# uzh-rpg/dagr

Measured on AMD Instinct MI355X. Metric: events_per_sec, higher is better.
Workload: dtype f32; 1 GPU; dagr-s + --use_image --img_net resnet50, 640x480 synthetic S-uniform, B=8 windows/step x 100000 events (50 ms each), r=7, K=16, events->graph->GNN(+image fusion)->decoded head outputs->confidence mask + NMS (device); image_branch=in-line, engines=3

## Files before the change

### dagr_amd/csrc/dense.hip

```cpp
#include "common.hpp"

namespace dagr {
namespace {

__global__ __launch_bounds__(kBlock) void k_dense_winner(const int32_t *__restrict__ n_ptr, int n_max,
                                                        const float *__restrict__ pos,
                                                        const int32_t *__restrict__ batch, float vx, float vy, int B,
                                                        int Hc, int Wc, int32_t *__restrict__ winner,
                                                        int32_t *__restrict__ status) {
    const int n_nodes = n_ptr ? min(*n_ptr, n_max) : n_max;
    const int n = blockIdx.x * kBlock + threadIdx.x;
    if (n >= n_nodes) return;
    const int cx = (int)(pos[3 * n] / vx), cy = (int)(pos[3 * n + 1] / vy), b = batch[n];
    if (cx < 0 || cx >= Wc || cy < 0 || cy >= Hc || b < 0 || b >= B) { atomicOr(status, 1); return; }
    atomicMax(&winner[(b * Hc + cy) * Wc + cx], n);
}

__global__ __launch_bounds__(kBlock) void k_dense_write(int B, int C, int Hc, int Wc,
                                                       const int32_t *__restrict__ winner,
                                                       const float *__restrict__ x, int ldx,
                                                       float *__restrict__ dense) {
    const int gid = blockIdx.x * kBlock + threadIdx.x;
    if (gid >= B * C * Hc * Wc) return;
    const int cx = gid % Wc, cy = (gid / Wc) % Hc, ch = (gid / (Wc * Hc)) % C, b = gid / (Wc * Hc * C);
// ... 69 lines not shown
namespace {
__global__ __launch_bounds__(kBlock) void k_bn_relu_maxpool(const float *__restrict__ x, int B, int H, int W, int C,
                                                           const float *__restrict__ scale,
                                                           const float *__restrict__ shift, float *__restrict__ y,
                                                           int OH, int OW) {
    const int C4 = C >> 2;
    const int64_t total = (int64_t)B * OH * OW * C4;
    const int64_t gid = (int64_t)blockIdx.x * kBlock + threadIdx.x;
    if (gid >= total) return;
    const int c4 = (int)(gid % C4);
    int64_t r = gid / C4;
    const int ow = (int)(r % OW); r /= OW;
    const int oh = (int)(r % OH);
    const int b = (int)(r / OH);
    const float4 sc = reinterpret_cast<const float4 *>(scale)[c4], sh = reinterpret_cast<const float4 *>(shift)[c4];
    float4 m = make_float4(0.f, 0.f, 0.f, 0.f);
#pragma unroll
    for (int dy = 0; dy < 3; dy++) {
        const int ih = 2 * oh - 1 + dy;
        if (ih < 0 || ih >= H) continue;
#pragma unroll
        for (int dx = 0; dx < 3; dx++) {
            const int iw = 2 * ow - 1 + dx;
            if (iw < 0 || iw >= W) continue;
            const float4 v = reinterpret_cast<const float4 *>(x + (((size_t)b * H + ih) * W + iw) * C)[c4];
            m.x = fmaxf(m.x, v.x * sc.x + sh.x);
            m.y = fmaxf(m.y, v.y * sc.y + sh.y);
            m.z = fmaxf(m.z, v.z * sc.z + sh.z);
            m.w = fmaxf(m.w, v.w * sc.w + sh.w);
        }
    }
    reinterpret_cast<float4 *>(y + (((size_t)b * OH + oh) * OW + ow) * C)[c4] = m;
}
}
}

extern "C" int dagr_bn_relu_maxpool(const float *x_nhwc, int32_t B, int32_t H, int32_t W, int32_t C, const float *scale,
                                    const float *shift, float *y_nhwc, void *stream) {
    using namespace dagr;
    DAGR_CHECK_ARG(B >= 1 && H >= 1 && W >= 1 && C >= 4 && C % 4 == 0, "bad sizes (C must be a multiple of 4)");
    DAGR_CHECK_ARG(x_nhwc && scale && shift && y_nhwc, "NULL pointer");
    DAGR_CHECK_ARG(((uintptr_t)x_nhwc % 16) == 0 && ((uintptr_t)y_nhwc % 16) == 0 && ((uintptr_t)scale % 16) == 0 &&
                       ((uintptr_t)shift % 16) == 0, "buffers must be 16-byte aligned");
    const int OH = (H - 1) / 2 + 1, OW = (W - 1) / 2 + 1;
    const int64_t total = (int64_t)B * OH * OW * (C / 4);
    k_bn_relu_maxpool<<<(unsigned)ceil_div(total, (int64_t)kBlock), kBlock, 0, (hipStream_t)stream>>>(
        x_nhwc, B, H, W, C, scale, shift, y_nhwc, OH, OW);
    DAGR_CHECK_LAUNCH();
    return DAGR_OK;
}

namespace dagr {
namespace {
__global__ __launch_bounds__(kBlock) void k_bias_relu(float *__restrict__ y, const float *__restrict__ bias, int64_t n4,
                                                     int C4) {
    const int64_t stride = (int64_t)gridDim.x * kBlock;
    for (int64_t i = (int64_t)blockIdx.x * kBlock + threadIdx.x; i < n4; i += stride) {
        float4 a = reinterpret_cast<float4 *>(y)[i];
        const float4 b = reinterpret_cast<const float4 *>(bias)[i % C4];
        a.x += b.x; a.y += b.y; a.z += b.z; a.w += b.w;
        a.x = a.x < 0.f ? 0.f : a.x;
        a.y = a.y < 0.f ? 0.f : a.y;
        a.z = a.z < 0.f ? 0.f : a.z;
        a.w = a.w < 0.f ? 0.f : a.w;
        reinterpret_cast<float4 *>(y)[i] = a;
    }
}
}
}

namespace dagr {
namespace {
__global__ __launch_bounds__(kBlock) void k_bias_silu(float *__restrict__ y, const float *__restrict__ bias, int64_t n4,
                                                     int C4) {
    const int64_t stride = (int64_t)gridDim.x * kBlock;
    for (int64_t i = (int64_t)blockIdx.x * kBlock + threadIdx.x; i < n4; i += stride) {
        float4 a = reinterpret_cast<float4 *>(y)[i];
        const float4 b = reinterpret_cast<const float4 *>(bias)[i % C4];
        a.x += b.x; a.y += b.y; a.z += b.z; a.w += b.w;
        a.x = a.x / (1.0f + expf(-a.x));
        a.y = a.y / (1.0f + expf(-a.y));
        a.z = a.z / (1.0f + expf(-a.z));
        a.w = a.w / (1.0f + expf(-a.w));
        reinterpret_cast<float4 *>(y)[i] = a;
    }
}
}
}

extern "C" int dagr_bias_silu(float *y_nhwc, const float *bias, int64_t n, int32_t C, void *stream) {
    using namespace dagr;
    DAGR_CHECK_ARG(n >= 0 && C >= 4 && C % 4 == 0 && n % C == 0, "bad sizes (C must be a multiple of 4 and divide n)");
    if (n == 0) return DAGR_OK;
    DAGR_CHECK_ARG(y_nhwc && bias, "NULL pointer");
    DAGR_CHECK_ARG(((uintptr_t)y_nhwc % 16) == 0 && ((uintptr_t)bias % 16) == 0, "buffers must be 16-byte aligned");
    const int64_t n4 = n >> 2;
    const int64_t blocks = ceil_div(n4, (int64_t)kBlock * 4);
    k_bias_silu<<<(unsigned)std::min<int64_t>(blocks, 256 * 16), kBlock, 0, (hipStream_t)stream>>>(y_nhwc, bias, n4, C / 4);
    DAGR_CHECK_LAUNCH();
    return DAGR_OK;
}

extern "C" int dagr_bias_relu(float *y_nhwc, const float *bias, int64_t n, int32_t C, void *stream) {
    using namespace dagr;
    DAGR_CHECK_ARG(n >= 0 && C >= 4 && C % 4 == 0 && n % C == 0, "bad sizes (C must be a multiple of 4 and divide n)");
    if (n == 0) return DAGR_OK;
// ... 9 lines not shown
```

### dagr_amd/csrc/gemm_lt.hip

```cpp
#include <hipblaslt/hipblaslt.h>

#include <map>
#include <tuple>

#include "common.hpp"

namespace dagr {
namespace {

struct LtPlan {
    hipblasLtMatmulDesc_t desc = nullptr;
    hipblasLtMatrixLayout_t a = nullptr, b = nullptr, c = nullptr, d = nullptr;
    hipblasLtMatmulAlgo_t algo;
    size_t workspace = 0;
};

hipblasLtHandle_t lt_handle() {
    static hipblasLtHandle_t h = [] {
        hipblasLtHandle_t hh = nullptr;
        if (hipblasLtCreate(&hh) != HIPBLAS_STATUS_SUCCESS) hh = nullptr;
        return hh;
    }();
    return h;
}

}
}

using namespace dagr;

extern "C" size_t dagr_gemm_epilogue_workspace_bytes(void) { return (size_t)64 << 20; }

extern "C" int dagr_gemm_epilogue(const float *A, int64_t M, int32_t K, int64_t lda, const float *Wt, int32_t N,
                                  const float *bias, const float *R, int64_t ldr, int32_t act, float *D, int64_t ldd,
                                  void *workspace, size_t workspace_bytes, void *stream) {
    DAGR_CHECK_ARG(M >= 0 && K >= 1 && N >= 1 && lda >= K && ldd >= N && (!R || ldr >= N) && (act == 0 || act == 1), "bad sizes");
    if (M == 0) return DAGR_OK;
    DAGR_CHECK_ARG(A && Wt && D, "NULL pointer");
    DAGR_CHECK_ARG((const float *)D != A, "D aliases A");
    DAGR_CHECK_ARG((const float *)D != R, "D aliases R");
    hipblasLtHandle_t h = lt_handle();
    if (!h) { set_error("dagr_gemm_epilogue: hipblasLtCreate failed"); return DAGR_ERR_HIP; }
    using Key = std::tuple<int64_t, int, int, int64_t, int64_t, int64_t, int, int, int>;
    static thread_local std::map<Key, LtPlan> plans;
    const Key key{M, K, N, lda, R ? ldr : -1, ldd, act, bias ? 1 : 0, R ? 1 : 0};
    auto it = plans.find(key);
    if (it == plans.end()) {
        LtPlan p;
#define LT_OK(expr)                                                                                        \
    do {                                                                                                   \
        if ((expr) != HIPBLAS_STATUS_SUCCESS) { set_error("dagr_gemm_epilogue: " #expr " failed"); return DAGR_ERR_HIP; } \
    } while (0)
        LT_OK(hipblasLtMatmulDescCreate(&p.desc, HIPBLAS_COMPUTE_32F, HIP_R_32F));
        const hipblasOperation_t op_n = HIPBLAS_OP_N;
        LT_OK(hipblasLtMatmulDescSetAttribute(p.desc, HIPBLASLT_MATMUL_DESC_TRANSA, &op_n, sizeof(op_n)));
        LT_OK(hipblasLtMatmulDescSetAttribute(p.desc, HIPBLASLT_MATMUL_DESC_TRANSB, &op_n, sizeof(op_n)));
        hipblasLtEpilogue_t epi = act ? (bias ? HIPBLASLT_EPILOGUE_RELU_BIAS : HIPBLASLT_EPILOGUE_RELU)
                                      : (bias ? HIPBLASLT_EPILOGUE_BIAS : HIPBLASLT_EPILOGUE_DEFAULT);
        LT_OK(hipblasLtMatmulDescSetAttribute(p.desc, HIPBLASLT_MATMUL_DESC_EPILOGUE, &epi, sizeof(epi)));
        if (bias) {
            const hipDataType bt = HIP_R_32F;
            LT_OK(hipblasLtMatmulDescSetAttribute(p.desc, HIPBLASLT_MATMUL_DESC_BIAS_DATA_TYPE, &bt, sizeof(bt)));
            LT_OK(hipblasLtMatmulDescSetAttribute(p.desc, HIPBLASLT_MATMUL_DESC_BIAS_POINTER, &bias, sizeof(bias)));
        }
        LT_OK(hipblasLtMatrixLayoutCreate(&p.a, HIP_R_32F, (uint64_t)N, (uint64_t)K, (int64_t)N));
        LT_OK(hipblasLtMatrixLayoutCreate(&p.b, HIP_R_32F, (uint64_t)K, (uint64_t)M, lda));
        LT_OK(hipblasLtMatrixLayoutCreate(&p.c, HIP_R_32F, (uint64_t)N, (uint64_t)M, R ? ldr : ldd));
        LT_OK(hipblasLtMatrixLayoutCreate(&p.d, HIP_R_32F, (uint64_t)N, (uint64_t)M, ldd));
        hipblasLtMatmulPreference_t pref = nullptr;
        LT_OK(hipblasLtMatmulPreferenceCreate(&pref));
        const uint64_t max_ws = workspace ? (uint64_t)workspace_bytes : 0;
        LT_OK(hipblasLtMatmulPreferenceSetAttribute(pref, HIPBLASLT_MATMUL_PREF_MAX_WORKSPACE_BYTES, &max_ws, sizeof(max_ws)));
        constexpr int kCand = 16;
        hipblasLtMatmulHeuristicResult_t res[kCand];
        int found = 0;
        const hipblasStatus_t st = hipblasLtMatmulAlgoGetHeuristic(h, p.desc, p.a, p.b, p.c, p.d, pref, kCand, res, &found);
        hipblasLtMatmulPreferenceDestroy(pref);
        if (st != HIPBLAS_STATUS_SUCCESS || found < 1) {
            set_error("dagr_gemm_epilogue: the library offers no kernel for this GEMM + epilogue");
            return DAGR_ERR_UNSUPPORTED;
        }
        int best = 0;
        hipStreamCaptureStatus cap = hipStreamCaptureStatusNone;
        (void)hipStreamIsCapturing((hipStream_t)stream, &cap);
        if (found > 1 && cap == hipStreamCaptureStatusNone) {
            hipEvent_t e0, e1;
            if (hipEventCreate(&e0) == hipSuccess && hipEventCreate(&e1) == hipSuccess) {
                const float alpha = 1.0f, beta = R ? 1.0f : 0.0f;
                float best_ms = 0.f;
                for (int c = 0; c < found; c++) {
                    if (res[c].workspaceSize > workspace_bytes) continue;
                    bool ok = true;
                    float ms = 0.f;
                    for (int rep = 0; rep < 3 && ok; rep++) {
                        if (rep == 1) (void)hipEventRecord(e0, (hipStream_t)stream);
                        ok = hipblasLtMatmul(h, p.desc, &alpha, Wt, p.a, A, p.b, &beta, R ? (const void *)R : (const void *)D,
                                             p.c, D, p.d, &res[c].algo, workspace, workspace_bytes,
                                             (hipStream_t)stream) == HIPBLAS_STATUS_SUCCESS;
                    }
                    (void)hipEventRecord(e1, (hipStream_t)stream);
                    if (hipEventSynchronize(e1) != hipSuccess || !ok) continue;
                    (void)hipEventElapsedTime(&ms, e0, e1);
                    if (best_ms == 0.f || ms < best_ms) { best_ms = ms; best = c; }
                }
                (void)hipEventDestroy(e0);
                (void)hipEventDestroy(e1);
            }
        }
        p.algo = res[best].algo;
        p.workspace = res[best].workspaceSize;
        it = plans.emplace(key, p).first;
#undef LT_OK
    }
    LtPlan &p = it->second;
    if (bias && hipblasLtMatmulDescSetAttribute(p.desc, HIPBLASLT_MATMUL_DESC_BIAS_POINTER, &bias, sizeof(bias)) !=
                    HIPBLAS_STATUS_SUCCESS) {
        set_error("dagr_gemm_epilogue: setting the bias pointer failed");
        return DAGR_ERR_HIP;
    }
    DAGR_CHECK_ARG(p.workspace <= workspace_bytes, "workspace too small for the selected kernel");
    const float alpha = 1.0f, beta = R ? 1.0f : 0.0f;
    const hipblasStatus_t st = hipblasLtMatmul(h, p.desc, &alpha, Wt, p.a, A, p.b, &beta, R ? (const void *)R : (const void *)D,
                                               p.c, D, p.d, &p.algo, workspace, workspace_bytes, (hipStream_t)stream);
    if (st != HIPBLAS_STATUS_SUCCESS) {
        set_error("dagr_gemm_epilogue: hipblasLtMatmul failed");
        return DAGR_ERR_HIP;
    }
    return DAGR_OK;
}
```

### dagr_amd/engine.py

```python
import contextlib
import ctypes
import gc
import types

import numpy as np
import torch

from . import _lib
from .graph.ev_graph import WindowGraphBuilder

FUSED_PASSES_MAX_NODES = 1600

L0_WIDTHS = (8, 16, 32)


def _l0_block(c):
    cm = max(b for b in (0,) + L0_WIDTHS if b <= c)
    return cm, c - cm


def _f32(v):
    return float(torch.as_tensor(v, dtype=torch.float32))


# ... 142 lines not shown


def _add_relu_(y, z):
    if y.is_cuda and y.dtype == torch.float32 and z.dtype == torch.float32 and y.shape == z.shape \
            and y.stride() == z.stride() and y.data_ptr() % 16 == 0 and z.data_ptr() % 16 == 0 \
            and (y.is_contiguous() or y.is_contiguous(memory_format=torch.channels_last)):
        _lib.check(_lib.lib().dagr_add_relu(_lib.ptr(y), _lib.ptr(z), y.numel(), _lib.cur_stream(y.device)), "add_relu")
        return y
    return torch.relu_(y.add_(z))


def _bias_relu_(y, bias):
    C = y.shape[1]
    if y.is_cuda and y.dtype == torch.float32 and C % 4 == 0 and y.is_contiguous(memory_format=torch.channels_last) \
            and y.data_ptr() % 16 == 0 and bias.data_ptr() % 16 == 0:
        _lib.check(_lib.lib().dagr_bias_relu(_lib.ptr(y), _lib.ptr(bias), y.numel(), C, _lib.cur_stream(y.device)),
                   "bias_relu")
        return y
    return torch.relu_(y.add_(bias.view(1, -1, 1, 1)))


def _baseconv_forward(m, x):
    y = m.conv(x)
    b = m._bias
    C = y.shape[1]
    if y.is_cuda and y.dtype == torch.float32 and C % 4 == 0 and y.is_contiguous(memory_format=torch.channels_last) \
            and y.data_ptr() % 16 == 0 and b.data_ptr() % 16 == 0:
        _lib.check(_lib.lib().dagr_bias_silu(_lib.ptr(y), _lib.ptr(b), y.numel(), C, _lib.cur_stream(y.device)),
                   "bias_silu")
        return y
    return torch.nn.functional.silu(y.add_(b.view(1, -1, 1, 1)), inplace=True)


def _conv_bias_relu(blk, name, x):
    conv = getattr(blk, name)
    b = getattr(blk, "_" + name + "_bias", None)
    out = conv(x)
    if b is not None:
        return _bias_relu_(out, b)
    if getattr(conv, "relu", False):
        return out
    return blk.relu(out)


def _bottleneck_forward(blk, x):
    identity = x if blk.downsample is None else blk.downsample(x)
    out = _conv_bias_relu(blk, "conv1", x)
    out = _conv_bias_relu(blk, "conv2", out)
    if isinstance(blk.conv3, _Conv1x1Gemm):
        return blk.conv3(out, residual=identity)
    return _add_relu_(blk.conv3(out), identity)


def _resnet_features_forward(net, x, emit=None):
    emit = emit or (lambda name, t: None)
    c1 = net.conv1(x)
    emit("conv1", c1)
    mp = net.maxpool
    ok = (c1.is_cuda and c1.dtype == torch.float32 and c1.is_contiguous(memory_format=torch.channels_last)
          and c1.shape[1] % 4 == 0 and mp.kernel_size == 3 and mp.stride == 2 and mp.padding == 1
          and mp.dilation == 1 and not mp.ceil_mode)
    if ok:
        B, C, H, W = c1.shape
        scale, shift = net._stem_affine
        y = torch.empty((B, C, (H - 1) // 2 + 1, (W - 1) // 2 + 1), dtype=c1.dtype, device=c1.device,
                        memory_format=torch.channels_last)
        _lib.check(_lib.lib().dagr_bn_relu_maxpool(_lib.ptr(c1), B, H, W, C, _lib.ptr(scale), _lib.ptr(shift), _lib.ptr(y),
                                                   _lib.cur_stream(c1.device)), "bn_relu_maxpool")
    else:
        y = net.maxpool(net.relu(net.bn1(c1)))
    l1 = net.layer1(y)
    emit("layer1", l1)
    l2 = net.layer2(l1)
    emit("layer2", l2)
    l3 = net.layer3(l2)
    emit("layer3", l3)
    l4 = net.layer4(l3)
    emit("layer4", l4)
    return dict(conv1=c1, layer1=l1, layer2=l2, layer3=l3, layer4=l4)


def _basicblock_forward(blk, x):
    identity = x if blk.downsample is None else blk.downsample(x)
    out = _conv_bias_relu(blk, "conv1", x)
    return _add_relu_(blk.conv2(out), identity)


class _Level:

    def __init__(self, T, cin, cout, device, cf_next=0):
        self.T = T
        self.e_cap = T * 64
        i32 = dict(dtype=torch.int32, device=device)
        f32 = dict(dtype=torch.float32, device=device)
        self.x = torch.zeros((T, (cin + 3) // 4 * 4), **f32)
        self.pos = torch.zeros((T, 3), **f32)
        self.batch = torch.zeros((T,), **i32)
        self.rowptr = torch.zeros((T + 2,), **i32)
        self.col = torch.zeros((self.e_cap,), **i32)
        self.code = torch.zeros((self.e_cap,), **i32)
        self.counts = torch.zeros((2,), **i32)
        self.cluster = torch.zeros((T,), **i32)
        self.h1 = torch.zeros((T, cout), **f32)
        self.hp = torch.zeros((T, cout + cf_next), **f32)
        self.cout = cout


class WindowEngine:
    def __init__(self, model, max_events=1 << 17, device="cuda"):
        self.model = model
        self.device = torch.device(device)
        args = model.args
        bb, head = model.backbone, model.head
        self.args = args
        self.B = int(args.batch_size)
        self.W, self.H = int(model.width), int(model.height)
        self.time_window = int(getattr(args, "time_window_us", 1000000))
        self.num_classes = bb.num_classes
        self.num_scales = int(args.num_scales)
        self.use_image = bool(args.use_image)
        self.no_events = bool(getattr(args, "no_events", False))
        self.feat_ch = list(bb.net.feature_channels) if self.use_image else [0] * 5
# ... 415 lines not shown

    def _fold_image_branch(self):
        import copy
        from torch.nn.utils.fusion import fuse_conv_bn_eval
        bb, head = self.model.backbone, self.model.head
        net = copy.deepcopy(bb.net).eval()
        cnn = copy.deepcopy(head.cnn_head).eval()

        def fold_block(blk):
            for ci, bi in (("conv1", "bn1"), ("conv2", "bn2"), ("conv3", "bn3")):
                if hasattr(blk, ci):
                    setattr(blk, ci, fuse_conv_bn_eval(getattr(blk, ci), getattr(blk, bi)))
                    setattr(blk, bi, torch.nn.Identity())
            if blk.downsample is not None:
                blk.downsample = torch.nn.Sequential(fuse_conv_bn_eval(blk.downsample[0], blk.downsample[1]))
        for name in ("layer1", "layer2", "layer3", "layer4"):
            for blk in getattr(net.module, name):
                fold_block(blk)
        for m in cnn.modules():
            if hasattr(m, "conv") and hasattr(m, "bn") and isinstance(m.bn, torch.nn.BatchNorm2d):
                m.conv = fuse_conv_bn_eval(m.conv, m.bn)
                m.bn = torch.nn.Identity()
                if isinstance(getattr(m, "act", None), torch.nn.SiLU) and m.conv.bias is not None:
                    m._bias = m.conv.bias.detach().clone().contiguous()
                    m.conv.bias = None
                    m.forward = types.MethodType(_baseconv_forward, m)
        net = net.to(memory_format=torch.channels_last)
        cnn = cnn.to(memory_format=torch.channels_last)
        for blkname in ("layer1", "layer2", "layer3", "layer4"):
            _gemmify_1x1(getattr(net.module, blkname))
            for blk in getattr(net.module, blkname):
                relu_convs = ("conv1", "conv2") if hasattr(blk, "conv3") else ("conv1",)
                for cname in relu_convs:
                    conv = getattr(blk, cname)
                    if isinstance(conv, _Conv1x1Gemm):
                        conv.relu = True
                    elif isinstance(conv, torch.nn.Conv2d) and conv.bias is not None:
                        setattr(blk, "_" + cname + "_bias", conv.bias.detach().clone().contiguous())
                        conv.bias = None
                blk.forward = types.MethodType(_bottleneck_forward if hasattr(blk, "conv3") else _basicblock_forward,
                                               blk)
        bn = net.module.bn1
        scale = (bn.weight.detach().float() / torch.sqrt(bn.running_var.detach().float() + bn.eps)).contiguous()
        shift = (bn.bias.detach().float() - bn.running_mean.detach().float() * scale).contiguous()
        net.module._stem_affine = (scale, shift)
        net.module.forward_features = types.MethodType(_resnet_features_forward, net.module)
        _gemmify_1x1(net.feature_dconv)
        _gemmify_1x1(net.output_dconv)
        self._net_f, self._cnn_f = net, cnn

    def _image_branch(self, image, on_feature=None):
        if self._net_f is None:
            self._fold_image_branch()
        bb, head = types.SimpleNamespace(net=self._net_f), types.SimpleNamespace(cnn_head=self._cnn_f)
        x = image.contiguous(memory_format=torch.channels_last)
        net = self._net_f
        if on_feature is not None:
            feats = [None] * len(net.feature_layers)

            def emit(name, t):
                if name in net.feature_layers:
                    j = net.feature_layers.index(name)
                    feats[j] = net.feature_dconv[j](t) if len(net.feature_dconv) > 0 else t
                    on_feature(j, feats[j])
            d = _resnet_features_forward(net.module, x, emit)
            outs = [d[l] for l in net.output_layers]
            if len(net.output_dconv) > 0:
                outs = [dconv(o) for o, dconv in zip(outs, net.output_dconv)]
        else:
            feats, outs = bb.net(x)
        outs = outs[-self.num_scales:]
        resized = [torch.nn.functional.interpolate(f, o) for f, o in zip(outs, self.out_sizes)]
        return feats, head.cnn_head(resized)

    def stage_image(self, image):
        self._keep = []
        self._img_feats, self._cnn_out = self._image_branch(image)

    def image_async(self, image, stream=None):
        cur = torch.cuda.current_stream(self.device)
        if stream is not None:
            self._img_stream = stream
        if self._img_stream is None:
            self._img_stream = torch.cuda.Stream(self.device)
        s = self._img_stream
        s.wait_stream(cur)
        with torch.cuda.stream(s):
            feats, cnn_out = self._image_branch(image)
            ev = torch.cuda.Event()
            ev.record(s)
        return feats, cnn_out, ev

    def _consume_image_handle(self, handle):
        feats, cnn_out, ev = handle
        cur = torch.cuda.current_stream(self.device)
        cur.wait_event(ev)
        for t in list(feats) + [o for v in cnn_out.values() for o in v]:
            t.record_stream(cur)
        self._keep = []
        self._img_feats, self._cnn_out = feats, cnn_out

    def stage_l0_input(self, feat):
        N = self._N
        x0 = self.x0buf[:N]
        g = self.graph
        if not self._inputs_gathered:
            f = feat.float().reshape(-1).contiguous()
            _lib.check(self.L.dagr_graph_gather_inputs(ctypes.byref(g.desc), _lib.ptr(g.workspace), _lib.ptr(self._pos),
                                                       _lib.ptr(f), N, _lib.ptr(self.pos_n), _lib.ptr(self.batch_n),
                                                       _lib.ptr(x0), self.x0_ld, self.x0_feat_col, self.x0_pos_col,
                                                       _lib.cur_stream(self.device)), "graph_gather_inputs")
        if self.use_image:
            self._sample(self._nptr(), N, self.pos_n, self.batch_n, 0, self._img_feats[0], x0, self.x0_img_col)
        self._x0 = x0

    def _conv_l0(self, pack, x, ldx, xskip, ldskip, out, ldo):
        L, P = self.L, _lib.ptr
        nbr_src, nbr_code, deg = self._nbr
        cin, cskip, w, s = pack
        d0 = self.dom[0]
        wx, tx, wy, ty = self.win0
        stream = _lib.cur_stream(self.device)
        if self.l0_tiles:
# ... 519 lines not shown
```

### include/dagr_hip.h

```cpp
#ifndef DAGR_HIP_H
#define DAGR_HIP_H

#include <stddef.h>
#include <stdint.h>

#ifdef __cplusplus
extern "C" {
#endif

typedef enum {
    DAGR_OK = 0,
    DAGR_ERR_INVALID_ARG = -1,
    DAGR_ERR_HIP = -2,
    DAGR_ERR_WORKSPACE = -3,
    DAGR_ERR_UNSUPPORTED = -4
} dagr_status;

const char *dagr_last_error(void);
int dagr_version(void);
int dagr_device_count(void);

int dagr_format_events(const int16_t *xy , const int32_t *t , const int8_t *p ,
                       int64_t N, int32_t width, int32_t height, int32_t time_window,
                       float *pos_out , float *feat_out , void *stream);
// ... 190 lines not shown
    const float *w2, *s2; float *hp0; int32_t ldhp0;
    const dagr_pool_desc *pdesc; void *pool_ws; const int32_t *xlo, *ylo;
    float *x_out; int32_t ldo; float *pos_out; int32_t *batch_out, *n_out, *rowptr_out, *col_out, *code_out, *e_out;
    int32_t e_cap;
} dagr_async_update_args;
int dagr_async_update(const dagr_async_update_args *args, void *stream);
int dagr_async_update_w(const dagr_async_update_args *args, int32_t cout0, void *stream);
int dagr_pool_l0_accumulate(const dagr_pool_desc *desc, void *pool_ws, const dagr_graph_desc *gdesc, void *graph_ws,
                            const int32_t *xlo, const int32_t *ylo, const float *x, int32_t ldx, const float *pos,
                            int64_t N, const int32_t *nbr_src, const int16_t *nbr_code, const int32_t *deg, void *stream);
int dagr_pool_l0_stream(const dagr_pool_desc *desc, void *pool_ws, int32_t rebuild, const dagr_graph_desc *gdesc,
                        void *graph_ws, const int32_t *xlo, const int32_t *ylo, const float *x, int32_t ldx, const float *pos,
                        const int32_t *batch_events, int64_t n_window, int64_t first_row, int64_t n_rows,
                        const int32_t *nbr_src, const int16_t *nbr_code, const int32_t *deg, float *x_out, int32_t ldo,
                        int32_t xoff, float *pos_out, int32_t *batch_out, int32_t *n_out, int32_t *rowptr_out,
                        int32_t *col_out, int32_t *code_out, int32_t *e_out, int32_t e_cap, void *stream);

int dagr_spline_conv_fused_pool(const int32_t *n_nodes_ptr, int32_t n_nodes_max, const int32_t *rowptr,
                                const int32_t *col, const int32_t *code, const float *x, int32_t ldx, int32_t cin,
                                const float *xskip, int32_t ldskip, int32_t cskip, int32_t rx, int32_t ry,
                                float den_x, float den_y, const float *Wq, const float *bias, float *C,
                                int32_t ldc, int32_t N, int32_t relu, const dagr_pool_desc *pdesc, void *pool_ws,
                                const float *pos, const int32_t *batch, int32_t *cluster_scratch, void *stream);
int dagr_pool_csr(const dagr_pool_desc *desc, void *pool_ws, const int32_t *n_ptr, int32_t n_max, const float *x,
                  int32_t ldx, const float *pos, const int32_t *batch, const int32_t *rowptr, const int32_t *col,
                  int32_t *cluster_scratch , float *x_out, int32_t ldo, int32_t xoff, float *pos_out,
                  int32_t *batch_out, int32_t *n_out, int32_t *rowptr_out, int32_t *col_out, int32_t *code_out,
                  int32_t *e_out, int32_t e_cap, void *stream);
int dagr_pool_recode(const int32_t *n_ptr, int32_t n_max, const int32_t *rowptr, const int32_t *col, const float *pos,
                     float two_max, float r00, float r02, float r11, float r12, int32_t rx, int32_t ry,
                     int32_t *code_out, int32_t e_cap, int32_t *status, void *stream);
int dagr_pool_status(const dagr_pool_desc *desc, void *pool_ws, int32_t *flags_host, void *stream);
const int32_t *dagr_pool_status_ptr(const dagr_pool_desc *desc, void *pool_ws);
int dagr_pool_counters(const dagr_pool_desc *desc, void *pool_ws, int32_t *out8_host, void *stream);

int dagr_to_dense(const int32_t *n_ptr, int32_t n_max, const float *x, int32_t ldx, int32_t channels,
                  const float *pos, const int32_t *batch, float vx, float vy, int32_t batch_size,
                  int32_t Hc, int32_t Wc, int32_t *winner_scratch, float *dense, int32_t *status, void *stream);

int dagr_pool_argmax(const int32_t *cluster, int32_t n, const float *x, int32_t ldx, int32_t channels,
                     const float *x_pooled, int32_t ldp, int32_t n_clusters, int32_t *arg, void *stream);
int dagr_pool_grad(const int32_t *cluster, int32_t n, int32_t channels, int32_t aggr, const int32_t *arg,
                   const int32_t *count, const float *grad_pooled, int32_t ldg, float *grad_x, int32_t ldgx,
                   void *stream);
int dagr_to_dense_grad(int32_t n, int32_t channels, const float *pos, const int32_t *batch, float vx, float vy,
                       int32_t batch_size, int32_t Hc, int32_t Wc, const float *grad_dense,
                       float *grad_x, int32_t ldgx, void *stream);

int dagr_add_relu(float *y, const float *z, int64_t n, void *stream);
int dagr_bias_relu(float *y_nhwc, const float *bias, int64_t n, int32_t C, void *stream);
int dagr_bias_silu(float *y_nhwc, const float *bias, int64_t n, int32_t C, void *stream);
int dagr_bn_relu_maxpool(const float *x_nhwc, int32_t B, int32_t H, int32_t W, int32_t C, const float *scale,
                         const float *shift, float *y_nhwc, void *stream);

int dagr_sample_features(const int32_t *n_ptr, int32_t n_max, const float *pos, const void *batch,
                         int32_t batch_is_int64, const float *feat_nhwc, int32_t B, int32_t h, int32_t w, int32_t C,
                         int32_t width, int32_t height, float *out, int32_t ldo, int32_t coff, void *stream);

int dagr_nms_batched(const float *boxes, const float *scores, const int32_t *cls, const uint8_t *valid,
                     int32_t B, int32_t A, float iou_threshold, float class_offset,
                     int32_t *order_out, int32_t *keep_out, int32_t *n_keep, void *stream);

typedef struct dagr_head_scale {
    const int32_t *n_ptr; int32_t n_max;
    const float *pred; int32_t ld;
    const float *pos; const int32_t *batch;
    float vx, vy, stride; int32_t Hc, Wc;
    const float *cnn[3]; int32_t cnn_stride[3][4];
    float *dense;
} dagr_head_scale;
int dagr_heads_finish(const dagr_head_scale *scale0, const dagr_head_scale *scale1, int32_t batch_size, int32_t channels,
                      float *out, int32_t *status, void *stream);
int dagr_heads_finish_detect(const dagr_head_scale *scale0, const dagr_head_scale *scale1, int32_t batch_size,
                             int32_t channels, float *out, int32_t *status, float conf_threshold, float iou_threshold,
                             float class_offset, float *det, int32_t *n_keep, void *stream);
int dagr_decode_heads(const float *dense0, int32_t H0, int32_t W0, float stride0, const float *dense1, int32_t H1,
                      int32_t W1, float stride1, int32_t B, int32_t channels, float *out, void *stream);

int dagr_postprocess(const float *pred, int32_t B, int32_t A, int32_t num_classes, float conf_threshold,
                     float iou_threshold, float class_offset, float *det, int32_t *n_keep, void *stream);

int dagr_masked_lin(const int64_t *indices, const float *x_in, float *x_out, const float *weight, const float *bias,
                    int32_t add, int64_t K, int32_t Cin, int32_t Cout, void *stream);
int dagr_masked_lin_no_bias(const int64_t *indices, const float *x_in, float *x_out, const float *weight, int32_t add,
                            int64_t K, int32_t Cin, int32_t Cout, void *stream);
int dagr_masked_isdiff(int64_t *indices, const float *x_old, const float *x_new, float atol, float rtol, int64_t K,
                       int32_t C, void *stream);
int dagr_masked_inplace_BN(const int64_t *indices, const float *x, float *x_out, const float *running_mean,
                           const float *running_var, const float *weight, const float *bias, float eps, int64_t K,
                           int32_t C, void *stream);

int dagr_downsample_events(const int32_t *order, const int32_t *run_cell, const int32_t *run_end, int32_t n_runs,
                           const int8_t *polarity, int32_t fx, int32_t fy, float *change_map, uint8_t *keep,
                           void *stream);

size_t dagr_gemm_epilogue_workspace_bytes(void);
int dagr_gemm_epilogue(const float *A, int64_t M, int32_t K, int64_t lda, const float *Wt, int32_t N, const float *bias,
                       const float *R, int64_t ldr, int32_t act, float *D, int64_t ldd, void *workspace,
                       size_t workspace_bytes, void *stream);

enum { DAGR_FLOPS_ZERO = 0, DAGR_FLOPS_CONV = 1, DAGR_FLOPS_LINEAR = 2, DAGR_FLOPS_POOL = 3, DAGR_FLOPS_CARTESIAN = 4 };
typedef struct dagr_flops_module {
    int32_t kind, level, cin, cout, root, bias;
} dagr_flops_module;
int dagr_async_flops(const int32_t *deg, int32_t n_events, const int32_t *counts1, const int32_t *counts2,
                     const int32_t *counts3, const int32_t *counts4, const dagr_flops_module *mods, int32_t n_mods,
                     int64_t *out, void *stream);

size_t dagr_viz_workspace_bytes(int32_t F, int32_t H, int32_t W);
int dagr_viz_render(const uint8_t *images, int32_t n_images, int32_t H, int32_t W, const int32_t *frame_image, int32_t F,
                    const int32_t *ev_x, const int32_t *ev_y, const int8_t *ev_p, const int32_t *ev_ptr, int32_t n_events,
                    const double *alpha, const int32_t *boxes, const int32_t *box_ptr, int32_t n_boxes, int32_t linewidth,
                    const uint8_t *colors, int32_t n_colors, uint8_t *out, int32_t *status, void *workspace,
                    size_t workspace_bytes, void *stream);

typedef struct dagr_aug_params {
    int32_t flip, crop_on;
    int32_t crop_lo[2], crop_hi[2];
    float zoom;
    int32_t move[2];
} dagr_aug_params;
size_t dagr_augment_workspace_bytes(int64_t N);
int dagr_augment_events(const dagr_aug_params *params, int32_t B, int32_t W, int32_t H, const void *pos, int32_t pos_width,
                        const void *t, int32_t t_width, const void *p, int32_t p_width, const int32_t *sample_ptr, int64_t N,
                        int16_t *out_pos, void *out_t, void *out_p, int64_t *out_batch, int32_t *out_ptr,
                        int32_t *status, void *workspace, size_t workspace_bytes, void *stream);
int dagr_augment_status(const int32_t *status, void *stream);
int dagr_augment_frames(const dagr_aug_params *params, int32_t B, int32_t C, int32_t H, int32_t W, int32_t elem_bytes,
                        int32_t reference_crop, const void *in, void *out, void *stream);
int dagr_augment_boxes(const dagr_aug_params *params, int32_t B, int32_t W, int32_t H, const float *boxes,
                       const int64_t *box_batch, int32_t M, int32_t ld, float *out, void *stream);

#define DAGR_COCO_MAX_GT 256
#define DAGR_COCO_MAX_DT 4096
#define DAGR_COCO_MAX_DETS 100
void dagr_coco_match_bounds(int32_t *max_gt, int32_t *max_dt, int32_t *max_dets);
int dagr_coco_match(const double *gt_xywh, const double *dt_xywh, const double *dt_score, const int64_t *jobs,
                    const double *area_rng, const double *iou_thrs, int32_t n_thr, int32_t max_dets, int64_t n_jobs,
                    int64_t n_gt, int64_t n_dt, int32_t max_gt_per_job, int32_t max_dt_per_job, int64_t n_out,
                    int64_t n_gign, int32_t *order, uint8_t *dtm, uint8_t *dt_ign, uint8_t *g_ign, int32_t *status,
                    void *stream);

#define DAGR_COCO_ACC_TILE 1024
#define DAGR_COCO_ACC_MAX_REC 128
int32_t dagr_coco_accumulate_tile(void);
size_t dagr_coco_accumulate_workspace_bytes(int32_t n_thr, int64_t n_cols);
int dagr_coco_accumulate(const uint8_t *dtm, const uint8_t *dt_ign, const int32_t *perm, const int64_t *group_ptr,
                         const int64_t *group_ngt, const double *rec_thrs, int32_t n_rec, double eps, int32_t n_thr,
                         int32_t n_groups, int64_t n_cols, void *workspace, size_t workspace_bytes, double *precision,
                         int32_t *status, void *stream);

int dagr_spiral_offsets(int32_t n, int32_t *dx_host, int32_t *dy_host);
// ... 6 lines not shown
```

Before: 147.5 million events/s.

## Fuse stem BN-ReLU-maxpool with conv1 projection and widen hipBLASLt algo search

New measurement: 148.4 million events/s, median of 6. About the same (+0.6%).

```diff
diff --git a/dagr_amd/csrc/dense.hip b/dagr_amd/csrc/dense.hip
--- a/dagr_amd/csrc/dense.hip
+++ b/dagr_amd/csrc/dense.hip
@@ -145,6 +145,169 @@
 
 namespace dagr {
 namespace {
+constexpr int kStemRows = 4, kStemCols = 32;
+constexpr int kStemLR = kStemRows + 1, kStemLC = kStemCols + 1;
+constexpr int kStemPix = kStemLR * kStemLC;
+constexpr int kStemMaxC = 64;
+constexpr int kStemLoads = (kStemPix * (kStemMaxC / 4) + kBlock - 1) / kBlock;
+
+template <int NT>
+__device__ __forceinline__ void stem_tile_compute(const float4 *l_x, const float4 *l_aff, int tile, int B, int H, int W,
+                                                  int C, float *__restrict__ y, int OH, int OW, const float *__restrict__ wd,
+                                                  const float *__restrict__ bd, int N, float *__restrict__ proj,
+                                                  int tiles_x, int tiles_y) {
+    const int C4 = C >> 2, ld4 = C4 + 1;
+    const int q_step = kBlock / C4, c_step = kBlock - q_step * C4;
+    const int q_first = (int)threadIdx.x / C4, c_first = (int)threadIdx.x - q_first * C4;
+    {
+        const int tx = tile % tiles_x, ty = (tile / tiles_x) % tiles_y, b = tile / (tiles_x * tiles_y);
+        const int r0 = ty * kStemRows - 1, c0 = tx * kStemCols - 1;
+
+        constexpr int kOwned = kStemRows * kStemCols;
+        for (int item = threadIdx.x; item < kOwned * (N / NT); item += kBlock) {
+            const int p = item & (kOwned - 1);
+            const int n0 = __builtin_amdgcn_readfirstlane(item / kOwned) * NT;
+            const int lr = 1 + p / kStemCols, lc = 1 + p % kStemCols;
+            const int ih = r0 + lr, iw = c0 + lc;
+            if (ih >= H || iw >= W) continue;
+            const float4 *src = l_x + (lr * kStemLC + lc) * ld4;
+            float acc[NT];
+#pragma unroll
+            for (int j = 0; j < NT; j++) acc[j] = 0.f;
+            for (int k4 = 0; k4 < C4; k4++) {
+                const float4 f = src[k4];
+                const float *w = wd + (size_t)(4 * k4) * N + n0;
+#pragma unroll
+                for (int j = 0; j < NT; j++) acc[j] = fmaf(f.x, w[j], acc[j]);
+#pragma unroll
+                for (int j = 0; j < NT; j++) acc[j] = fmaf(f.y, w[N + j], acc[j]);
+#pragma unroll
+                for (int j = 0; j < NT; j++) acc[j] = fmaf(f.z, w[2 * N + j], acc[j]);
+#pragma unroll
+                for (int j = 0; j < NT; j++) acc[j] = fmaf(f.w, w[3 * N + j], acc[j]);
+            }
+            float *out = proj + (((size_t)b * H + ih) * W + iw) * N + n0;
+#pragma unroll
+            for (int j = 0; j < NT; j += 4)
+                reinterpret_cast<float4 *>(out)[j >> 2] = make_float4(acc[j] + bd[n0 + j], acc[j + 1] + bd[n0 + j + 1],
+                                                                      acc[j + 2] + bd[n0 + j + 2], acc[j + 3] + bd[n0 + j + 3]);
+        }
+
+        constexpr int kPoolCols = kStemCols / 2, kPooled = (kStemRows / 2) * kPoolCols;
+        int q = q_first, c4 = c_first;
+        for (; q < kPooled; q += q_step) {
+            const int ohl = q / kPoolCols, owl = q % kPoolCols;
+            const int oh = ty * (kStemRows / 2) + ohl, ow = tx * kPoolCols + owl;
+            if (oh < OH && ow < OW) {
+                const float4 sc = l_aff[c4], sh = l_aff[C4 + c4];
+                float4 m = make_float4(0.f, 0.f, 0.f, 0.f);
+#pragma unroll
+                for (int dy = 0; dy < 3; dy++) {
+                    const int ih = 2 * oh - 1 + dy;
+#pragma unroll
+                    for (int dx = 0; dx < 3; dx++) {
+                        const int iw = 2 * ow - 1 + dx;
+                        const bool in = ih >= 0 && ih < H && iw >= 0 && iw < W;
+                        const float4 f = l_x[((2 * ohl + dy) * kStemLC + 2 * owl + dx) * ld4 + c4];
+                        m.x = fmaxf(m.x, in ? f.x * sc.x + sh.x : 0.f);
+                        m.y = fmaxf(m.y, in ? f.y * sc.y + sh.y : 0.f);
+                        m.z = fmaxf(m.z, in ? f.z * sc.z + sh.z : 0.f);
+                        m.w = fmaxf(m.w, in ? f.w * sc.w + sh.w : 0.f);
+                    }
+                }
+                reinterpret_cast<float4 *>(y + (((size_t)b * OH + oh) * OW + ow) * C)[c4] = m;
+            }
+            c4 += c_step;
+            if (c4 >= C4) { c4 -= C4; q++; }
+        }
+    }
+}
+
+template <int NT>
+__global__ __launch_bounds__(kBlock) void k_stem_tail(const float *__restrict__ x, int B, int H, int W, int C,
+                                                     const float *__restrict__ scale, const float *__restrict__ shift,
+                                                     float *__restrict__ y, int OH, int OW,
+                                                     const float *__restrict__ wd, const float *__restrict__ bd, int N,
+                                                     float *__restrict__ proj, int tiles_x, int tiles_y, int n_tiles) {
+    extern __shared__ float4 l_x[];
+    const int C4 = C >> 2, ld4 = C4 + 1;
+    const int q_step = kBlock / C4, c_step = kBlock - q_step * C4;
+    const int q_first = (int)threadIdx.x / C4, c_first = (int)threadIdx.x - q_first * C4;
+    const XcdSplit sp = xcd_split(n_tiles, 1, 0);
+    float4 *l_aff = l_x + kStemPix * ld4 + 1;
+    if ((int)threadIdx.x < 2 * C4)
+        l_aff[threadIdx.x] = (int)threadIdx.x < C4 ? reinterpret_cast<const float4 *>(scale)[threadIdx.x]
+                                                   : reinterpret_cast<const float4 *>(shift)[threadIdx.x - C4];
+
+    static_assert(kStemLoads == 11, "STEM_EACH lists the loads of a tile");
+#define STEM_EACH(OP) OP(0) OP(1) OP(2) OP(3) OP(4) OP(5) OP(6) OP(7) OP(8) OP(9) OP(10)
+#define STEM_DECL(u) float4 v##u = make_float4(0.f, 0.f, 0.f, 0.f); int dst##u = 0;
+    STEM_EACH(STEM_DECL)
+    int tile = -1, next = sp.first;
+    while (true) {
+        const bool more = next < sp.end;
+        if (more) {
+            const int tx = next % tiles_x, ty = (next / tiles_x) % tiles_y, b = next / (tiles_x * tiles_y);
+            const int r0 = ty * kStemRows - 1, c0 = tx * kStemCols - 1;
+            const float *xb = x + (size_t)b * H * W * C;
+            int px = q_first, c4 = c_first;
+#define STEM_LOAD(u)                                                                                  \
+            {                                                                                         \
+                const int pxc = min(px, kStemPix - 1);                                                \
+                const int lr = pxc / kStemLC, lc = pxc - lr * kStemLC;                                \
+                const int ih = r0 + lr, iw = c0 + lc;                                                 \
+                const bool keep = px < kStemPix && ih >= 0 && ih < H && iw >= 0 && iw < W;            \
+                const int ihc = min(max(ih, 0), H - 1), iwc = min(max(iw, 0), W - 1);                 \
+                v##u = reinterpret_cast<const float4 *>(xb + ((size_t)ihc * W + iwc) * C)[c4];        \
+                dst##u = keep ? pxc * ld4 + c4 : kStemPix * ld4;                                      \
+                px += q_step;                                                                         \
+                c4 += c_step;                                                                         \
+                if (c4 >= C4) { c4 -= C4; px++; }                                                     \
+            }
+            STEM_EACH(STEM_LOAD)
+#undef STEM_LOAD
+        }
+        if (tile >= 0) stem_tile_compute<NT>(l_x, l_aff, tile, B, H, W, C, y, OH, OW, wd, bd, N, proj, tiles_x, tiles_y);
+        if (!more) break;
+        __syncthreads();
+#define STEM_STAGE(u) l_x[dst##u] = v##u;
+        STEM_EACH(STEM_STAGE)
+#undef STEM_STAGE
+        __syncthreads();
+        tile = next;
+        next += sp.stride;
+    }
+#undef STEM_DECL
+#undef STEM_EACH
+}
+}
+}
+
+extern "C" int dagr_stem_tail(const float *x_nhwc, int32_t B, int32_t H, int32_t W, int32_t C, const float *scale,
+                              const float *shift, float *y_nhwc, const float *wd, const float *bd, int32_t N,
+                              float *proj_nhwc, void *stream) {
+    using namespace dagr;
+    DAGR_CHECK_ARG(B >= 1 && H >= 1 && W >= 1 && C >= 4 && C % 4 == 0 && C <= kStemMaxC && N >= 4 && N % 4 == 0 && N <= 64,
+                   "bad sizes (C and N must be multiples of 4, at most 64)");
+    DAGR_CHECK_ARG(x_nhwc && scale && shift && y_nhwc && wd && bd && proj_nhwc, "NULL pointer");
+    for (const void *p : {(const void *)x_nhwc, (const void *)scale, (const void *)shift, (const void *)y_nhwc,
+                          (const void *)wd, (const void *)bd, (const void *)proj_nhwc})
+        DAGR_CHECK_ARG(((uintptr_t)p % 16) == 0, "buffers must be 16-byte aligned");
+    const int OH = (H - 1) / 2 + 1, OW = (W - 1) / 2 + 1;
+    const int tiles_y = (int)ceil_div(OH, kStemRows / 2), tiles_x = (int)ceil_div(OW, kStemCols / 2);
+    const int64_t n_tiles = (int64_t)B * tiles_y * tiles_x;
+    DAGR_CHECK_ARG(n_tiles < (1ll << 31) - 8, "map too large");
+    const size_t lds = ((size_t)kStemPix * (C / 4 + 1) + 1 + 2 * (C / 4)) * sizeof(float4);
+    auto kern = N % 8 == 0 ? k_stem_tail<8> : k_stem_tail<4>;
+    const unsigned grid = round_grid8(std::min<int64_t>(n_tiles, (int64_t)persistent_grid(kern, kBlock, lds, 1 << 30)));
+    kern<<<grid, kBlock, lds, (hipStream_t)stream>>>(x_nhwc, B, H, W, C, scale, shift, y_nhwc, OH, OW, wd, bd, N, proj_nhwc,
+                                                     tiles_x, tiles_y, (int)n_tiles);
+    DAGR_CHECK_LAUNCH();
+    return DAGR_OK;
+}
+
+namespace dagr {
+namespace {
 __global__ __launch_bounds__(kBlock) void k_bias_relu(float *__restrict__ y, const float *__restrict__ bias, int64_t n4,
                                                      int C4) {
     const int64_t stride = (int64_t)gridDim.x * kBlock;
diff --git a/dagr_amd/csrc/gemm_lt.hip b/dagr_amd/csrc/gemm_lt.hip
--- a/dagr_amd/csrc/gemm_lt.hip
+++ b/dagr_amd/csrc/gemm_lt.hip
@@ -1,7 +1,13 @@
+#include <hipblaslt/hipblaslt-ext.hpp>
 #include <hipblaslt/hipblaslt.h>
 
+#include <string.h>
+
+#include <algorithm>
+#include <chrono>
 #include <map>
 #include <tuple>
+#include <vector>
 
 #include "common.hpp"
 
@@ -13,7 +19,26 @@
     hipblasLtMatrixLayout_t a = nullptr, b = nullptr, c = nullptr, d = nullptr;
     hipblasLtMatmulAlgo_t algo;
     size_t workspace = 0;
+    int index = -1;
+    int screened = -1;
+    int from_search = 0;
+    float us = 0.f;
 };
+
+constexpr double kSearchMinFlop = 2e9;
+constexpr double kSearchBudgetMs = 1500.0;
+constexpr int kMaxSurvivors = 24;
+constexpr float kScreenSlack = 1.3f;
+
+using LtKey = std::tuple<int64_t, int, int, int64_t, int64_t, int64_t, int, int, int>;
+std::map<LtKey, LtPlan> &lt_plans() {
+    static thread_local std::map<LtKey, LtPlan> plans;
+    return plans;
+}
+int64_t &lt_search_count() {
+    static thread_local int64_t n = 0;
+    return n;
+}
 
 hipblasLtHandle_t lt_handle() {
     static hipblasLtHandle_t h = [] {
@@ -41,9 +66,8 @@
     DAGR_CHECK_ARG((const float *)D != R, "D aliases R");
     hipblasLtHandle_t h = lt_handle();
     if (!h) { set_error("dagr_gemm_epilogue: hipblasLtCreate failed"); return DAGR_ERR_HIP; }
-    using Key = std::tuple<int64_t, int, int, int64_t, int64_t, int64_t, int, int, int>;
-    static thread_local std::map<Key, LtPlan> plans;
-    const Key key{M, K, N, lda, R ? ldr : -1, ldd, act, bias ? 1 : 0, R ? 1 : 0};
+    std::map<LtKey, LtPlan> &plans = lt_plans();
+    const LtKey key{M, K, N, lda, R ? ldr : -1, ldd, act, bias ? 1 : 0, R ? 1 : 0};
     auto it = plans.find(key);
     if (it == plans.end()) {
         LtPlan p;
@@ -80,35 +104,71 @@
             set_error("dagr_gemm_epilogue: the library offers no kernel for this GEMM + epilogue");
             return DAGR_ERR_UNSUPPORTED;
         }
+        std::vector<hipblasLtMatmulHeuristicResult_t> cand(res, res + found);
         int best = 0;
         hipStreamCaptureStatus cap = hipStreamCaptureStatusNone;
         (void)hipStreamIsCapturing((hipStream_t)stream, &cap);
-        if (found > 1 && cap == hipStreamCaptureStatusNone) {
-            hipEvent_t e0, e1;
-            if (hipEventCreate(&e0) == hipSuccess && hipEventCreate(&e1) == hipSuccess) {
+        hipEvent_t e0, e1;
+        if (cap == hipStreamCaptureStatusNone && hipEventCreate(&e0) == hipSuccess) {
+            if (hipEventCreate(&e1) == hipSuccess) {
                 const float alpha = 1.0f, beta = R ? 1.0f : 0.0f;
-                float best_ms = 0.f;
-                for (int c = 0; c < found; c++) {
-                    if (res[c].workspaceSize > workspace_bytes) continue;
+                auto time_algo = [&](hipblasLtMatmulAlgo_t &algo, int warm, int timed) -> float {
                     bool ok = true;
-                    float ms = 0.f;
-                    for (int rep = 0; rep < 3 && ok; rep++) {
-                        if (rep == 1) (void)hipEventRecord(e0, (hipStream_t)stream);
+                    for (int rep = 0; rep < warm + timed && ok; rep++) {
+                        if (rep == warm) (void)hipEventRecord(e0, (hipStream_t)stream);
                         ok = hipblasLtMatmul(h, p.desc, &alpha, Wt, p.a, A, p.b, &beta, R ? (const void *)R : (const void *)D,
-                                             p.c, D, p.d, &res[c].algo, workspace, workspace_bytes,
+                                             p.c, D, p.d, &algo, workspace, workspace_bytes,
                                              (hipStream_t)stream) == HIPBLAS_STATUS_SUCCESS;
                     }
                     (void)hipEventRecord(e1, (hipStream_t)stream);
-                    if (hipEventSynchronize(e1) != hipSuccess || !ok) continue;
-                    (void)hipEventElapsedTime(&ms, e0, e1);
-                    if (best_ms == 0.f || ms < best_ms) { best_ms = ms; best = c; }
+                    float ms = 0.f;
+                    if (hipEventSynchronize(e1) != hipSuccess || !ok || hipEventElapsedTime(&ms, e0, e1) != hipSuccess) return -1.f;
+                    return ms;
+                };
+                if (2.0 * (double)M * (double)N * (double)K >= kSearchMinFlop) {
+                    std::vector<hipblasLtMatmulHeuristicResult_t> all;
+                    if (hipblaslt_ext::getAllAlgos(h, hipblaslt_ext::GemmType::HIPBLASLT_GEMM, op_n, op_n, HIP_R_32F, HIP_R_32F,
+                                                   HIP_R_32F, HIP_R_32F, HIPBLAS_COMPUTE_32F, all) != HIPBLAS_STATUS_SUCCESS)
+                        all.clear();
+                    lt_search_count()++;
+                    p.screened = 0;
+                    std::vector<std::pair<float, size_t>> kept;
+                    float best_ms = 0.f;
+                    const auto t0 = std::chrono::steady_clock::now();
+                    for (size_t c = 0; c < all.size(); c++) {
+                        if (std::chrono::duration<double, std::milli>(std::chrono::steady_clock::now() - t0).count() >
+                            kSearchBudgetMs)
+                            break;
+                        size_t need = 0;
+                        if (hipblaslt_ext::matmulIsAlgoSupported(h, p.desc, &alpha, p.a, p.b, &beta, p.c, p.d, all[c].algo,
+                                                                 need) != HIPBLAS_STATUS_SUCCESS || need > workspace_bytes)
+                            continue;
+                        all[c].workspaceSize = need;
+                        const float ms = time_algo(all[c].algo, 1, 1);
+                        p.screened++;
+                        if (ms <= 0.f || (best_ms > 0.f && ms > kScreenSlack * best_ms)) continue;
+                        if (best_ms == 0.f || ms < best_ms) best_ms = ms;
+                        kept.emplace_back(ms, c);
+                    }
+                    std::sort(kept.begin(), kept.end());
+                    for (size_t i = 0; i < kept.size() && (int)i < kMaxSurvivors; i++)
+                        if (kept[i].first <= kScreenSlack * best_ms) cand.push_back(all[kept[i].second]);
                 }
-                (void)hipEventDestroy(e0);
+                float best_ms = 0.f;
+                for (int c = 0; c < (int)cand.size(); c++) {
+                    if (cand[c].workspaceSize > workspace_bytes) continue;
+                    const float ms = cand.size() > 1 ? time_algo(cand[c].algo, 1, 2) : -1.f;
+                    if (ms > 0.f && (best_ms == 0.f || ms < best_ms)) { best_ms = ms; best = c; }
+                }
+                p.us = best_ms * 500.f;
                 (void)hipEventDestroy(e1);
             }
+            (void)hipEventDestroy(e0);
         }
-        p.algo = res[best].algo;
-        p.workspace = res[best].workspaceSize;
+        p.algo = cand[best].algo;
+        p.workspace = cand[best].workspaceSize;
+        p.index = hipblaslt_ext::getIndexFromAlgo(p.algo);
+        p.from_search = best >= found ? 1 : 0;
         it = plans.emplace(key, p).first;
 #undef LT_OK
     }
@@ -128,3 +188,25 @@
     }
     return DAGR_OK;
 }
+
+extern "C" int64_t dagr_gemm_epilogue_search_count(void) { return lt_search_count(); }
+
+extern "C" int64_t dagr_gemm_epilogue_report(char *buf, int64_t cap) {
+    std::string out;
+    for (const auto &kv : lt_plans()) {
+        const LtKey &k = kv.first;
+        const LtPlan &p = kv.second;
+        char line[256];
+        snprintf(line, sizeof(line), "%lld %d %d %lld %lld %lld %d %d %d -> index %d us %.1f screened %d wide %d\n",
+                 (long long)std::get<0>(k), std::get<1>(k), std::get<2>(k), (long long)std::get<3>(k),
+                 (long long)std::get<4>(k), (long long)std::get<5>(k), std::get<6>(k), std::get<7>(k), std::get<8>(k),
+                 p.index, p.us, p.screened, p.from_search);
+        out += line;
+    }
+    if (buf && cap > 0) {
+        const size_t n = std::min<size_t>(out.size(), (size_t)cap - 1);
+        memcpy(buf, out.data(), n);
+        buf[n] = 0;
+    }
+    return (int64_t)out.size();
+}
diff --git a/dagr_amd/engine.py b/dagr_amd/engine.py
--- a/dagr_amd/engine.py
+++ b/dagr_amd/engine.py
@@ -218,10 +218,9 @@
     return _add_relu_(blk.conv3(out), identity)
 
 
-def _resnet_features_forward(net, x, emit=None):
-    emit = emit or (lambda name, t: None)
+def _resnet_features_forward(net, x, emit=None, stem_dconv=None):
+    emit = emit or (lambda name, t, projected=None: None)
     c1 = net.conv1(x)
-    emit("conv1", c1)
     mp = net.maxpool
     ok = (c1.is_cuda and c1.dtype == torch.float32 and c1.is_contiguous(memory_format=torch.channels_last)
           and c1.shape[1] % 4 == 0 and mp.kernel_size == 3 and mp.stride == 2 and mp.padding == 1
@@ -231,9 +230,19 @@
         scale, shift = net._stem_affine
         y = torch.empty((B, C, (H - 1) // 2 + 1, (W - 1) // 2 + 1), dtype=c1.dtype, device=c1.device,
                         memory_format=torch.channels_last)
-        _lib.check(_lib.lib().dagr_bn_relu_maxpool(_lib.ptr(c1), B, H, W, C, _lib.ptr(scale), _lib.ptr(shift), _lib.ptr(y),
-                                                   _lib.cur_stream(c1.device)), "bn_relu_maxpool")
+        N = stem_dconv.wt.shape[1] if isinstance(stem_dconv, _Conv1x1Gemm) and stem_dconv.stride == 1 else 0
+        if C <= 64 and 4 <= N <= 64 and N % 4 == 0 and stem_dconv.wt.shape[0] == C and not stem_dconv.relu:
+            f0 = torch.empty((B, H, W, N), dtype=c1.dtype, device=c1.device)
+            _lib.check(_lib.lib().dagr_stem_tail(_lib.ptr(c1), B, H, W, C, _lib.ptr(scale), _lib.ptr(shift), _lib.ptr(y),
+                                                 _lib.ptr(stem_dconv.wt), _lib.ptr(stem_dconv.b), N, _lib.ptr(f0),
+                                                 _lib.cur_stream(c1.device)), "stem_tail")
+            emit("conv1", c1, f0.permute(0, 3, 1, 2))
+        else:
+            emit("conv1", c1)
+            _lib.check(_lib.lib().dagr_bn_relu_maxpool(_lib.ptr(c1), B, H, W, C, _lib.ptr(scale), _lib.ptr(shift),
+                                                       _lib.ptr(y), _lib.cur_stream(c1.device)), "bn_relu_maxpool")
     else:
+        emit("conv1", c1)
         y = net.maxpool(net.relu(net.bn1(c1)))
     l1 = net.layer1(y)
     emit("layer1", l1)
@@ -755,23 +764,26 @@
     def _image_branch(self, image, on_feature=None):
         if self._net_f is None:
             self._fold_image_branch()
-        bb, head = types.SimpleNamespace(net=self._net_f), types.SimpleNamespace(cnn_head=self._cnn_f)
+        head = types.SimpleNamespace(cnn_head=self._cnn_f)
         x = image.contiguous(memory_format=torch.channels_last)
         net = self._net_f
-        if on_feature is not None:
-            feats = [None] * len(net.feature_layers)
-
-            def emit(name, t):
-                if name in net.feature_layers:
-                    j = net.feature_layers.index(name)
+        feats = [None] * len(net.feature_layers)
+
+        def emit(name, t, projected=None):
+            if name in net.feature_layers:
+                j = net.feature_layers.index(name)
+                if projected is not None:
+                    feats[j] = projected
+                else:
                     feats[j] = net.feature_dconv[j](t) if len(net.feature_dconv) > 0 else t
+                if on_feature is not None:
                     on_feature(j, feats[j])
-            d = _resnet_features_forward(net.module, x, emit)
-            outs = [d[l] for l in net.output_layers]
-            if len(net.output_dconv) > 0:
-                outs = [dconv(o) for o, dconv in zip(outs, net.output_dconv)]
-        else:
-            feats, outs = bb.net(x)
+        stem = net.feature_dconv[0] if (len(net.feature_dconv) > 0 and net.feature_layers[:1] == ["conv1"]
+                                        and net.feature_layers.count("conv1") == 1) else None
+        d = _resnet_features_forward(net.module, x, emit, stem_dconv=stem)
+        outs = [d[l] for l in net.output_layers]
+        if len(net.output_dconv) > 0:
+            outs = [dconv(o) for o, dconv in zip(outs, net.output_dconv)]
         outs = outs[-self.num_scales:]
         resized = [torch.nn.functional.interpolate(f, o) for f, o in zip(outs, self.out_sizes)]
         return feats, head.cnn_head(resized)
diff --git a/include/dagr_hip.h b/include/dagr_hip.h
--- a/include/dagr_hip.h
+++ b/include/dagr_hip.h
@@ -266,6 +266,9 @@
 int dagr_bias_silu(float *y_nhwc, const float *bias, int64_t n, int32_t C, void *stream);
 int dagr_bn_relu_maxpool(const float *x_nhwc, int32_t B, int32_t H, int32_t W, int32_t C, const float *scale,
                          const float *shift, float *y_nhwc, void *stream);
+int dagr_stem_tail(const float *x_nhwc, int32_t B, int32_t H, int32_t W, int32_t C, const float *scale,
+                   const float *shift, float *y_nhwc, const float *wd, const float *bd, int32_t N, float *proj_nhwc,
+                   void *stream);
 
 int dagr_sample_features(const int32_t *n_ptr, int32_t n_max, const float *pos, const void *batch,
                          int32_t batch_is_int64, const float *feat_nhwc, int32_t B, int32_t h, int32_t w, int32_t C,
@@ -312,6 +315,8 @@
 int dagr_gemm_epilogue(const float *A, int64_t M, int32_t K, int64_t lda, const float *Wt, int32_t N, const float *bias,
                        const float *R, int64_t ldr, int32_t act, float *D, int64_t ldd, void *workspace,
                        size_t workspace_bytes, void *stream);
+int64_t dagr_gemm_epilogue_search_count(void);
+int64_t dagr_gemm_epilogue_report(char *buf, int64_t cap);
 
 enum { DAGR_FLOPS_ZERO = 0, DAGR_FLOPS_CONV = 1, DAGR_FLOPS_LINEAR = 2, DAGR_FLOPS_POOL = 3, DAGR_FLOPS_CARTESIAN = 4 };
 typedef struct dagr_flops_module {
```
